# jeffersonfparil/poolgen

Hardware: AMD Instinct MI355X
Metric: loci/sec ols_iter_with_kinship, 200 pools x 10M loci (higher is better)
Workload: dtype f64

## Files before the change

### poolgen_amd/csrc/pg_kinship.hip

```cpp
#include "pg_common.h"
#include <cstdlib>
#include <cstring>
#include <utility>

namespace {

#ifndef KIN_WAVES_DEF
#define KIN_WAVES_DEF 16
#endif
constexpr int KIN_WAVES = KIN_WAVES_DEF;
constexpr int KIN_THREADS = 64 * KIN_WAVES;
#ifndef KIN_RING_D
#define KIN_RING_D 3
#endif
constexpr int KIN_FUSE_MAXK = 2;
constexpr int KIN_TPW = 96 / KIN_WAVES;
#ifndef KIN_KC_DEF
#define KIN_KC_DEF 16
#endif
constexpr int KIN_KC = KIN_KC_DEF;
constexpr int KIN_PPT = (KIN_KC * 128 + KIN_THREADS - 1) / KIN_THREADS;

typedef double double4_t __attribute__((ext_vector_type(4)));
typedef unsigned int uint4_t __attribute__((ext_vector_type(4)));

template <int CTRL, int ROW_MASK>
__device__ __forceinline__ double dpp_add(double v) {
    const int lo = __builtin_amdgcn_update_dpp(0, __double2loint(v), CTRL, ROW_MASK, 0xf, true);
    const int hi = __builtin_amdgcn_update_dpp(0, __double2hiint(v), CTRL, ROW_MASK, 0xf, true);
    return v + __hiloint2double(hi, lo);
}
template <int N>
__device__ __forceinline__ double row_from_plus(double v) {
    static_assert(N >= 1 && N <= 15, "row rotation");
    constexpr int CTRL = 0x120 + (16 - N);
    const int lo = __builtin_amdgcn_update_dpp(0, __double2loint(v), CTRL, 0xf, 0xf, false);
    const int hi = __builtin_amdgcn_update_dpp(0, __double2hiint(v), CTRL, 0xf, 0xf, false);
    return __hiloint2double(hi, lo);
}
template <int... I, typename F>
__device__ __forceinline__ void static_for_impl(std::integer_sequence<int, I...>, F &&f) {
    (f(std::integral_constant<int, I>{}), ...);
}
template <int N, typename F>
__device__ __forceinline__ void static_for(F &&f) {
    static_for_impl(std::make_integer_sequence<int, N>{}, f);
}
constexpr int kin_tri_ti(int t, int T) { int ti = 0; while (ti < T && t >= T - ti) { t -= T - ti; ++ti; } return ti < T ? ti : 0; }
constexpr int kin_tri_tj(int t, int T) { int ti = 0; while (ti < T && t >= T - ti) { t -= T - ti; ++ti; } return ti < T ? ti + t : 0; }
constexpr int kin_slot_tile(int w, int u, int T) { return (w + KIN_WAVES_DEF * u) < T * (T + 1) / 2 ? (w + KIN_WAVES_DEF * u) : 0; }

constexpr int KIN13_T[16][6][2] = {
    {{0, 0}, {0, 1}, {0, 2}, {1, 1}, {1, 2}, {2, 2}},
    {{3, 3}, {3, 4}, {3, 5}, {4, 4}, {4, 5}, {5, 5}},
    {{6, 6}, {6, 7}, {6, 8}, {7, 7}, {7, 8}, {8, 8}},
    {{9, 9}, {9, 10}, {9, 11}, {10, 10}, {10, 11}, {11, 11}},
    {{0, 3}, {0, 4}, {0, 5}, {1, 3}, {1, 4}, {1, 5}},
    {{0, 6}, {0, 7}, {0, 8}, {1, 6}, {1, 7}, {1, 8}},
    {{0, 9}, {0, 10}, {0, 11}, {1, 9}, {1, 10}, {1, 11}},
    {{3, 6}, {3, 7}, {3, 8}, {4, 6}, {4, 7}, {4, 8}},
    {{3, 9}, {3, 10}, {3, 11}, {4, 9}, {4, 10}, {4, 11}},
    {{6, 9}, {6, 10}, {6, 11}, {7, 9}, {7, 10}, {7, 11}},
    {{2, 4}, {2, 11}, {2, 12}, {4, 12}, {11, 12}, {12, 12}},
    {{2, 5}, {2, 6}, {2, 7}, {5, 6}, {5, 7}, {-1, -1}},
    {{0, 12}, {2, 3}, {3, 12}, {6, 12}, {7, 12}, {-1, -1}},
    {{5, 9}, {5, 10}, {5, 12}, {9, 12}, {10, 12}, {-1, -1}},
    {{2, 8}, {2, 9}, {2, 10}, {8, 9}, {8, 10}, {-1, -1}},
    {{1, 12}, {5, 8}, {5, 11}, {8, 11}, {8, 12}, {-1, -1}},
};
constexpr int kin13_ntiles(int w) { int c = 0; for (int u = 0; u < 6; ++u) c += KIN13_T[w][u][0] >= 0; return c; }
constexpr int kin13_col(int w, int idx) {
    int seen[12] = {-1, -1, -1, -1, -1, -1, -1, -1, -1, -1, -1, -1}, ns = 0;
    for (int u = 0; u < 6; ++u)
        for (int h = 0; h < 2; ++h) {
            const int c = KIN13_T[w][u][h];
            if (c < 0) continue;
            bool dup = false;
            for (int i = 0; i < ns; ++i) dup = dup || seen[i] == c;
            if (!dup) seen[ns++] = c;
        }
    return idx < ns ? seen[idx] : -1;
}
constexpr int kin13_ncols(int w) { int c = 0; while (c < 12 && kin13_col(w, c) >= 0) ++c; return c; }
constexpr int kin13_slot(int w, int col) { int i = 0; while (kin13_col(w, i) != col) ++i; return i; }
constexpr int KIN13_MAXC = 6;
constexpr int kin13_ndiag(int w) { int c = 0; for (int u = 0; u < 6; ++u) c += (KIN13_T[w][u][0] >= 0 && KIN13_T[w][u][0] == KIN13_T[w][u][1]); return c; }
constexpr int kin13_diag_index(int w, int u) { int c = 0; for (int v = 0; v < u; ++v) c += (KIN13_T[w][v][0] >= 0 && KIN13_T[w][v][0] == KIN13_T[w][v][1]); return c; }

struct KinParams {
    const double *G;
    int64_t p;
    int64_t ld;
    int64_t loci_per_wg;
    double *slabs;
    int n, T, npad, Tb, nb;
    int split;
    int merged;
    const double *ytil;
    double *spec;
    int k;
    int xcd_spx, npairs, nslab;
    int skip_dead;
    int wq_n[6], wq_first[6];
    int64_t wq_len[6];
};

template <bool FUSE, bool SPEC13, int SMALL = 0, bool SKIP = false>
__global__ __launch_bounds__(KIN_THREADS, 1) void k_kinship_syrk(KinParams P) {
    extern __shared__ __attribute__((aligned(16))) double lds[];
    const int tid = threadIdx.x;
    const int lane = tid & 63;
    const int wave = tid >> 6;
    const int fi = lane & 15;
    const int kq = lane >> 4;

    int bx = blockIdx.x, by = blockIdx.y;
    if (P.xcd_spx) {
        const int xcd = blockIdx.x & 7, s = blockIdx.x >> 3, main = P.xcd_spx * P.npairs;
        if (s < main) { bx = xcd * P.xcd_spx + s / P.npairs; by = s % P.npairs; }
        else { const int e = (s - main) * 8 + xcd; bx = 8 * P.xcd_spx + e / P.npairs; by = e % P.npairs; }
        if (bx >= P.nslab) return;
    }
    int64_t loci_per_wg = P.loci_per_wg;
    if (P.wq_n[0] > 0) {
        int q = 0;
        while (q + 1 < P.npairs && (int)blockIdx.x >= P.wq_first[q + 1]) ++q;
        by = q;
        bx = (int)blockIdx.x - P.wq_first[q];
        loci_per_wg = P.wq_len[q];
    }
    int bi = 0, bj = 0;
    {
        int q = by / P.split;
        const int first = P.merged ? 1 : 0;
        for (bi = 0; bi < P.nb; ++bi) {
            const int cnt = P.nb - bi - first;
            if (q < cnt) { bj = bi + first + q; break; }
            q -= cnt;
        }
    }
    const bool diag = (bi == bj);
    const int Ta = min(P.Tb, P.T - bi * P.Tb);
    const int Tbb = min(P.Tb, P.T - bj * P.Tb);
    const int colsA = Ta * 16;
    const int colsB = diag ? 0 : Tbb * 16;
    int ldsld = colsA + colsB;
    if ((ldsld & 31) != 16) ldsld += 16;
    const int a0 = bi * P.Tb * 16;
    const int b0 = bj * P.Tb * 16;
    const int wa = min(colsA, P.n - a0);
    const int wb = diag ? 0 : min(colsB, P.n - b0);
    const int npa = (wa + 1) >> 1, npb = (wb + 1) >> 1;
    const int npr = npa + npb;

    const int nrect = diag ? 0 : Ta * Tbb;
    const int NA = Ta * (Ta + 1) / 2, NB = Tbb * (Tbb + 1) / 2, part = P.nb - 1;
    const int rankA = bj - 1, rankB = bi;
    const int cntA = P.merged ? (NA > rankA ? (NA - rankA + part - 1) / part : 0) : 0;
    const int cntB = P.merged ? (NB > rankB ? (NB - rankB + part - 1) / part : 0) : 0;
    const int ntiles = diag ? NA : nrect + cntA + cntB;
    const int split_id = by % P.split;
    int acol[KIN_TPW], bcol[KIN_TPW], orow[KIN_TPW], ocol[KIN_TPW];
    bool live[KIN_TPW];
#pragma unroll
    for (int u = 0; u < KIN_TPW; ++u) {
        const int t = split_id + P.split * (wave + KIN_WAVES * u);
        int ti = 0, tj = 0;
        live[u] = t < ntiles;
        int kind = diag ? 1 : 0;
        if (t < ntiles) {
            int q = t, Td = Ta;
            if (!diag && t >= nrect) {
                const bool inA = t - nrect < cntA;
                kind = inA ? 1 : 2;
                q = inA ? rankA + part * (t - nrect) : rankB + part * (t - nrect - cntA);
                Td = inA ? Ta : Tbb;
            }
            if (kind) {
                for (ti = 0; ti < Td; ++ti) {
                    const int cnt = Td - ti;
                    if (q < cnt) { tj = ti + q; break; }
                    q -= cnt;
                }
            } else {
                ti = t / Tbb;
                tj = t - ti * Tbb;
            }
        }
        acol[u] = (kind == 2 ? colsA : 0) + 16 * ti;
        bcol[u] = (kind == 1 ? 0 : colsA) + 16 * tj;
        orow[u] = (kind == 2 ? b0 : a0) + 16 * ti;
        ocol[u] = (kind == 1 ? a0 : b0) + 16 * tj;
    }

    int st_loc[KIN_PPT], st_lcol[KIN_PPT];
    int st_gcol[KIN_PPT];
    bool st_on[KIN_PPT], st_two[KIN_PPT];
#pragma unroll
    for (int r = 0; r < KIN_PPT; ++r) {
        const int t = tid + r * KIN_THREADS;
        const int loc = t / npr;
        const int q = t - loc * npr;
        st_on[r] = loc < KIN_KC;
        st_loc[r] = loc;
        int gcol, lcol;
        bool two;
        if (q < npa) {
            gcol = a0 + 2 * q; lcol = 2 * q; two = (2 * q + 1) < wa;
        } else {
            const int q2 = q - npa;
            gcol = b0 + 2 * q2; lcol = colsA + 2 * q2; two = (2 * q2 + 1) < wb;
        }
        st_lcol[r] = lcol;
        st_two[r] = two;
        st_gcol[r] = st_on[r] ? gcol : a0;
        if (!st_on[r]) st_loc[r] = 0;
    }

    const int64_t l_begin = (int64_t)bx * loci_per_wg;
    const int64_t l_end = min(P.p, l_begin + loci_per_wg);
    const int nstages = (l_end > l_begin) ? (int)((l_end - l_begin + KIN_KC - 1) / KIN_KC) : 0;
    const int bufsz = KIN_KC * ldsld;

    for (int i = tid; i < 2 * bufsz; i += KIN_THREADS) lds[i] = 0.0;
    double *ylds = lds + 2 * bufsz;
    if (FUSE)
        for (int i = tid; i < P.k * 256; i += KIN_THREADS) ylds[i] = P.ytil[i];
    __syncthreads();

    const uint64_t slab_bytes64 = (uint64_t)(l_end > l_begin ? l_end - l_begin : 0) * P.ld * 8;
    const __amdgpu_buffer_rsrc_t rsrc = __builtin_amdgcn_make_buffer_rsrc(
        const_cast<double *>(P.G + l_begin * P.ld), 0, (int)(uint32_t)slab_bytes64, 0x00020000);
    uint4_t stage_reg[KIN_PPT];
    uint32_t st_voff[KIN_PPT];
#pragma unroll
    for (int r = 0; r < KIN_PPT; ++r)
        st_voff[r] = st_on[r] ? (uint32_t)(((int64_t)st_loc[r] * P.ld + st_gcol[r]) * 8) : 0xFFFFFFF0u;
    const uint32_t stage_stride = (uint32_t)(KIN_KC * P.ld * 8);
    auto stage_load = [&](int c) {
#pragma unroll
        for (int r = 0; r < KIN_PPT; ++r)
            stage_reg[r] = __builtin_amdgcn_raw_buffer_load_b128(
                rsrc, st_on[r] ? st_voff[r] + (uint32_t)c * stage_stride : 0xFFFFFFF0u, 0, 0);
    };
    auto stage_store = [&](int buf) {
#pragma unroll
        for (int r = 0; r < KIN_PPT; ++r) {
            if (st_on[r]) {
                uint4_t v = stage_reg[r];
                if (!st_two[r]) { v.z = 0u; v.w = 0u; }
                *reinterpret_cast<uint4_t *>(&lds[buf * bufsz + st_loc[r] * ldsld + st_lcol[r]]) = v;
            }
        }
    };

    if (nstages > 0) {
        stage_load(0);
        stage_store(0);
    }
    __syncthreads();

    const int NV = 2 + P.k;
    double *scratch = ylds + KIN_FUSE_MAXK * 256 + wave * (4 * 64);
    double yreg[KIN_FUSE_MAXK][4];
#pragma unroll
    for (int t = 0; t < KIN_FUSE_MAXK; ++t)
#pragma unroll
        for (int j = 0; j < 4; ++j) yreg[t][j] = (FUSE && t < P.k) ? ylds[t * 256 + lane + 64 * j] : 0.0;
    auto spec_pass = [&](const double *buf, int64_t lbase) {
#pragma unroll
        for (int jl = 0; jl < KIN_KC / KIN_WAVES; ++jl) {
            const int loc = wave + KIN_WAVES * jl;
            const double *row = buf + loc * ldsld;
            const double shift = row[0];
            double s1 = 0.0, s2 = 0.0, sy[KIN_FUSE_MAXK], d[4];
#pragma unroll
            for (int t = 0; t < KIN_FUSE_MAXK; ++t) sy[t] = 0.0;
#pragma unroll
            for (int j = 0; j < 4; ++j) {
                const int pool = lane + 64 * j;
                if (SPEC13 && j < 3) d[j] = row[pool] - shift;
                else {
                    const double gv = row[pool < ldsld ? pool : ldsld - 1];
                    d[j] = (pool < P.n) ? gv - shift : 0.0;
                }
                s1 += d[j];
                s2 = fma(d[j], d[j], s2);
                sy[0] = fma(d[j], yreg[0][j], sy[0]);
            }
            const bool two = P.k > 1;
            if (two) {
#pragma unroll
                for (int j = 0; j < 4; ++j) sy[1] = fma(d[j], yreg[1][j], sy[1]);
            }
            scratch[lane] = s1;
            scratch[64 + lane] = s2;
            scratch[2 * 64 + lane] = sy[0];
            if (two) scratch[3 * 64 + lane] = sy[1];
            __builtin_amdgcn_wave_barrier();
            const int v = lane >> 4, r = lane & 15;
            const double *sc = scratch + v * 64 + r;
            double tot = (sc[0] + sc[16]) + (sc[32] + sc[48]);
            tot = dpp_add<0x111, 0xf>(tot);
            tot = dpp_add<0x112, 0xf>(tot);
            tot = dpp_add<0x114, 0xf>(tot);
            tot = dpp_add<0x118, 0xf>(tot);
            const int64_t l = lbase + loc;
            if (r == 15 && v < NV && l < l_end) P.spec[l * NV + v] = tot;
            __builtin_amdgcn_wave_barrier();
        }
    };

    auto run = [&](auto wc, auto tc) {
        constexpr int W = decltype(wc)::value;
        constexpr int TPW = decltype(tc)::value;
        constexpr int KS = KIN_KC / 4;
        constexpr int NQ = KS * TPW;
        constexpr int D = KIN_RING_D, R = KIN_RING_D + 1;
        static_assert(NQ % R == 0 && NQ > 2 * D, "ring indexing assumes the stage length is a multiple of the ring");
        double4_t acc[TPW];
#pragma unroll
        for (int u = 0; u < TPW; ++u) acc[u] = (double4_t){0.0, 0.0, 0.0, 0.0};
#ifndef KIN_SHARED_FRAGS
#define KIN_SHARED_FRAGS 1
#endif
        if constexpr (W >= 0 && KIN_SHARED_FRAGS) {
            constexpr int NC = kin13_ncols(W), NT = kin13_ntiles(W);
            static_assert(NC <= KIN13_MAXC && KS % 2 == 0, "fragment sets alternate with the k-step parity");
            double fr[2][KIN13_MAXC];
            const double *lb = lds + kq * ldsld + fi;
            constexpr bool has_strip = [] { bool h = false; for (int u = 0; u < 6; ++u) h = h || (KIN13_T[W][u][0] >= 0 && KIN13_T[W][u][0] < 12 && KIN13_T[W][u][1] == 12); return h; }();
            double bs[2][2];
            const double *lbs = lds + kq * ldsld + 192 + (lane & 3);
            constexpr int ND = (SMALL & 1) ? kin13_ndiag(W) : 0;
            double bd[2][ND > 0 ? ND : 1][2];
            const double *lbr1 = lds + kq * ldsld + ((fi + 4) & 15), *lbr2 = lds + kq * ldsld + ((fi + 8) & 15);
            auto load_set = [&](const double *bufbase, auto sc, auto pc) __attribute__((always_inline)) {
                constexpr int s2 = decltype(sc)::value, par = decltype(pc)::value;
                static_for<NC>([&](auto cc) __attribute__((always_inline)) {
                    constexpr int ci = decltype(cc)::value;
                    fr[par][ci] = bufbase[4 * s2 * 208 + 16 * kin13_col(W, ci)];
                });
                if constexpr ((SMALL & 2) != 0 && has_strip) {
                    const double *bb = lbs + (bufbase - lb);
                    bs[par][0] = bb[4 * s2 * 208];
                    bs[par][1] = bb[4 * s2 * 208 + 4];
                }
                if constexpr (ND > 0) {
                    static_for<NT>([&](auto uc) __attribute__((always_inline)) {
                        constexpr int u = decltype(uc)::value;
                        if constexpr (KIN13_T[W][u][0] == KIN13_T[W][u][1]) {
                            constexpr int di = kin13_diag_index(W, u);
                            bd[par][di][0] = (lbr1 + (bufbase - lb))[4 * s2 * 208 + 16 * KIN13_T[W][u][0]];
                            bd[par][di][1] = (lbr2 + (bufbase - lb))[4 * s2 * 208 + 16 * KIN13_T[W][u][0]];
                        }
                    });
                }
            };
            auto mfma_set = [&](auto pc) __attribute__((always_inline)) {
                constexpr int par = decltype(pc)::value;
                static_for<NT>([&](auto uc) __attribute__((always_inline)) {
                    constexpr int u = decltype(uc)::value;
                    constexpr int ti = KIN13_T[W][u][0], tj = KIN13_T[W][u][1];
                    const double fa = fr[par][kin13_slot(W, ti)];
                    if constexpr ((SMALL & 1) != 0 && ti == tj) {
                        acc[u][0] = __builtin_amdgcn_mfma_f64_4x4x4f64(fa, fa, acc[u][0], 0, 0, 0);
                        acc[u][1] = __builtin_amdgcn_mfma_f64_4x4x4f64(fa, bd[par][kin13_diag_index(W, u)][0], acc[u][1], 0, 0, 0);
                        acc[u][2] = __builtin_amdgcn_mfma_f64_4x4x4f64(fa, bd[par][kin13_diag_index(W, u)][1], acc[u][2], 0, 0, 0);
                    } else if constexpr ((SMALL & 2) != 0 && tj == 12 && ti != tj) {
                        acc[u][0] = __builtin_amdgcn_mfma_f64_4x4x4f64(fa, bs[par][0], acc[u][0], 0, 0, 0);
                        acc[u][1] = __builtin_amdgcn_mfma_f64_4x4x4f64(fa, bs[par][1], acc[u][1], 0, 0, 0);
                    } else {
                        acc[u] = __builtin_amdgcn_mfma_f64_16x16x4f64(fa, fr[par][kin13_slot(W, tj)], acc[u], 0, 0, 0);
                    }
                });
            };
            if (nstages > 0) load_set(lb, std::integral_constant<int, 0>{}, std::integral_constant<int, 0>{});
            constexpr int spec_step = (W / 4) % KS;
            for (int c = 0; c < nstages; ++c) {
                const bool more = (c + 1) < nstages;
                if (more) stage_load(c + 1);
                const double *buf = lds + (c & 1) * bufsz;
                const double *b0 = lb + (c & 1) * bufsz;
                const double *b1 = lb + ((c + 1) & 1) * bufsz;
                static_for<KS>([&](auto sc) __attribute__((always_inline)) {
                    constexpr int s2 = decltype(sc)::value;
                    if constexpr (FUSE && s2 == spec_step) spec_pass(buf, l_begin + (int64_t)c * KIN_KC);
                    if constexpr (s2 + 1 < KS) {
                        load_set(b0, std::integral_constant<int, s2 + 1>{}, std::integral_constant<int, (s2 + 1) & 1>{});
                    } else {
                        if (more) stage_store((c + 1) & 1);
                        __syncthreads();
                        if (more) load_set(b1, std::integral_constant<int, 0>{}, std::integral_constant<int, 0>{});
                    }
                    mfma_set(std::integral_constant<int, s2 & 1>{});
                });
            }
            double *slab = P.slabs + (size_t)bx * P.npad * P.npad;
            static_for<NT>([&](auto uc) __attribute__((always_inline)) {
                constexpr int u = decltype(uc)::value;
                constexpr int ti = KIN13_T[W][u][0], tj = KIN13_T[W][u][1];
                constexpr int r0 = 16 * ti, c0 = 16 * tj;
                const int bi = lane >> 4, bb = (lane >> 2) & 3, bj = lane & 3;
                if constexpr ((SMALL & 1) != 0 && ti == tj) {
                    slab[(size_t)(r0 + 4 * bb + bi) * P.npad + c0 + 4 * bb + bj] = acc[u][0];
                    if (bb < 3) slab[(size_t)(r0 + 4 * bb + bi) * P.npad + c0 + 4 * (bb + 1) + bj] = acc[u][1];
                    else slab[(size_t)(r0 + bj) * P.npad + c0 + 12 + bi] = acc[u][1];
                    if (bb < 2) slab[(size_t)(r0 + 4 * bb + bi) * P.npad + c0 + 4 * (bb + 2) + bj] = acc[u][2];
                } else if constexpr ((SMALL & 2) != 0 && tj == 12 && ti != tj) {
                    slab[(size_t)(r0 + 4 * bb + bi) * P.npad + c0 + bj] = acc[u][0];
                    slab[(size_t)(r0 + 4 * bb + bi) * P.npad + c0 + 4 + bj] = acc[u][1];
                } else {
#pragma unroll
                    for (int r = 0; r < 4; ++r) slab[(size_t)(r0 + kq + 4 * r) * P.npad + c0 + fi] = acc[u][r];
                }
            });
            return;
        }
        double fa[R], fb[R];
        const double *lanebase = lds + kq * ldsld + fi;
        auto frag_load = [&](const double *bufbase, auto qc) {
            constexpr int q = decltype(qc)::value;
            constexpr int s = q / TPW, u = q % TPW;
            if constexpr (W >= 0) {
                if constexpr (W + KIN_WAVES * u >= 91) return;
                constexpr int t = kin_slot_tile(W, u, 13);
                constexpr int ao = 4 * s * 208 + 16 * kin_tri_ti(t, 13);
                constexpr int bo = 4 * s * 208 + 16 * kin_tri_tj(t, 13);
                fa[q % R] = bufbase[ao];
#ifdef KIN_EXP_HALF
                fb[q % R] = fa[q % R];
                (void)bo;
#elif defined(KIN_EXP_QUARTER)
                if constexpr (q % 2 == 0) fa[q % R] = bufbase[ao]; else fa[q % R] = fa[(q + R - 1) % R];
                fb[q % R] = fa[q % R];
                (void)bo;
#else
                fb[q % R] = bufbase[bo];
#endif
            } else {
                if constexpr (SKIP) { if (!live[u]) return; }
                const double *row = bufbase + 4 * s * ldsld;
                fa[q % R] = row[acol[u]];
                fb[q % R] = row[bcol[u]];
            }
        };
        auto mfma_item = [&](auto qc) {
            constexpr int q = decltype(qc)::value;
            constexpr int u = q % TPW;
            if constexpr (W >= 0 && W + KIN_WAVES * u >= 91) return;
            if constexpr (W < 0 && SKIP) { if (!live[u]) return; }
            acc[u] = __builtin_amdgcn_mfma_f64_16x16x4f64(fa[q % R], fb[q % R], acc[u], 0, 0, 0);
        };
        if (nstages > 0)
            static_for<D>([&](auto qc) { frag_load(lanebase, qc); });
        for (int c = 0; c < nstages; ++c) {
            const bool more = (c + 1) < nstages;
            if (more) stage_load(c + 1);
            const double *buf = lds + (c & 1) * bufsz;
            const double *fb0 = lanebase + (c & 1) * bufsz;
            const double *fb1 = lanebase + ((c + 1) & 1) * bufsz;
#ifndef KIN_SPEC_STAGGER
#define KIN_SPEC_STAGGER 1
#endif
            constexpr int spec_at = (FUSE && W >= 0 && KIN_SPEC_STAGGER) ? ((W / 4) % 4) * ((NQ - D) / 4) : -1;
            static_for<NQ - D>([&](auto qc) {
                if constexpr (decltype(qc)::value == spec_at) spec_pass(buf, l_begin + (int64_t)c * KIN_KC);
                frag_load(fb0, std::integral_constant<int, decltype(qc)::value + D>{});
                mfma_item(qc);
            });
            if (more) stage_store((c + 1) & 1);
            if (FUSE && spec_at < 0) spec_pass(buf, l_begin + (int64_t)c * KIN_KC);
            __syncthreads();
            static_for<D>([&](auto dc) {
                constexpr int q = NQ - D + decltype(dc)::value;
                if (more) frag_load(fb1, std::integral_constant<int, q + D - NQ>{});
                mfma_item(std::integral_constant<int, q>{});
            });
        }
        double *slab = P.slabs + (size_t)bx * P.npad * P.npad;
        static_for<TPW>([&](auto uc) {
            constexpr int u = decltype(uc)::value;
            bool on;
            int r0, c0;
            if constexpr (W >= 0) {
                constexpr int t = W + KIN_WAVES * u;
                on = t < 91;
                r0 = 16 * kin_tri_ti(kin_slot_tile(W, u, 13), 13);
                c0 = 16 * kin_tri_tj(kin_slot_tile(W, u, 13), 13);
            } else {
                on = live[u]; r0 = orow[u]; c0 = ocol[u];
            }
            if (on) {
#pragma unroll
                for (int r = 0; r < 4; ++r) slab[(size_t)(r0 + kq + 4 * r) * P.npad + c0 + fi] = acc[u][r];
            }
        });
    };
    if constexpr (SPEC13) {
        switch (wave) {
        case 0: run(std::integral_constant<int, 0>{}, std::integral_constant<int, KIN_TPW>{}); break;
        case 1: run(std::integral_constant<int, 1>{}, std::integral_constant<int, KIN_TPW>{}); break;
        case 2: run(std::integral_constant<int, 2>{}, std::integral_constant<int, KIN_TPW>{}); break;
        case 3: run(std::integral_constant<int, 3>{}, std::integral_constant<int, KIN_TPW>{}); break;
        case 4: run(std::integral_constant<int, 4>{}, std::integral_constant<int, KIN_TPW>{}); break;
        case 5: run(std::integral_constant<int, 5>{}, std::integral_constant<int, KIN_TPW>{}); break;
        case 6: run(std::integral_constant<int, 6>{}, std::integral_constant<int, KIN_TPW>{}); break;
#if KIN_WAVES_DEF == 8
        default: run(std::integral_constant<int, 7>{}, std::integral_constant<int, KIN_TPW>{}); break;
#else
        case 7: run(std::integral_constant<int, 7>{}, std::integral_constant<int, KIN_TPW>{}); break;
        case 8: run(std::integral_constant<int, 8>{}, std::integral_constant<int, KIN_TPW>{}); break;
        case 9: run(std::integral_constant<int, 9>{}, std::integral_constant<int, KIN_TPW>{}); break;
        case 10: run(std::integral_constant<int, 10>{}, std::integral_constant<int, KIN_TPW>{}); break;
        case 11: run(std::integral_constant<int, 11>{}, std::integral_constant<int, KIN_TPW>{}); break;
        case 12: run(std::integral_constant<int, 12>{}, std::integral_constant<int, KIN_TPW>{}); break;
        case 13: run(std::integral_constant<int, 13>{}, std::integral_constant<int, KIN_TPW>{}); break;
        case 14: run(std::integral_constant<int, 14>{}, std::integral_constant<int, KIN_TPW>{}); break;
        default: run(std::integral_constant<int, 15>{}, std::integral_constant<int, KIN_TPW>{}); break;
#endif
        }
    } else {
        constexpr std::integral_constant<int, -1> any{};
        switch ((ntiles + KIN_WAVES - 1) / KIN_WAVES) {
        case 0: case 1: case 2: run(any, std::integral_constant<int, 2>{}); break;
        case 3: run(any, std::integral_constant<int, 3>{}); break;
        case 4: run(any, std::integral_constant<int, 4>{}); break;
        case 5: run(any, std::integral_constant<int, 5>{}); break;
        default: run(any, std::integral_constant<int, KIN_TPW>{}); break;
        }
    }
}

constexpr double KIN_PAIR_FLOOR = 2.7;
struct KinCounts { int blk, nb, n[6]; };
__global__ __launch_bounds__(256) void k_kinship_reduce(const double *__restrict__ slabs, int nslabs, int npad, int n,
                                                        double add_const, double *__restrict__ S, const KinCounts C) {
    __shared__ double part[4][64];
    const int jj = threadIdx.x & 63, grp = threadIdx.x >> 6;
    const int j = blockIdx.x * 64 + jj;
    const int i = blockIdx.y;
    const bool on = i < n && j < n && i <= j;
    double s = 0.0;
    if (on && C.blk) {
        const int bi = i / C.blk, bj = j / C.blk;
        nslabs = C.n[bi * C.nb - bi * (bi - 1) / 2 + (bj - bi)];
    }
    if (on) {
        const size_t off = (size_t)i * npad + j;
        const size_t stride = (size_t)npad * npad;
        for (int w = grp; w < nslabs; w += 4) s += slabs[w * stride + off];
    }
    part[grp][jj] = s;
    __syncthreads();
    if (on && grp == 0) {
        const double t = ((part[0][jj] + part[1][jj]) + (part[2][jj] + part[3][jj])) + add_const;
        S[(size_t)i * n + j] = t;
        S[(size_t)j * n + i] = t;
    }
}

}

#ifndef KIN_LAUNCH_NAME
#define KIN_LAUNCH_NAME pg_launch_kinship
#endif
int KIN_LAUNCH_NAME(pg_ctx *ctx, const double *G, int64_t p, int n, int64_t ld, double *S,
                      bool add_intercept, int kid, bool allow_fuse) {
#if KIN_WAVES_DEF == 16
    if (n <= 64) return pg_launch_kinship_w8(ctx, G, p, n, ld, S, add_intercept, kid, allow_fuse);
#endif

    PG_CHECK(ctx, G && S, "kinship: null pointer");
    PG_CHECK(ctx, p > 0 && n > 0, "kinship: need p > 0 and n > 0 (p=%lld n=%d)", (long long)p, n);
    PG_CHECK(ctx, ld >= n && (ld % 2) == 0, "kinship: ld (%lld) must be even and >= n (%d)",
             (long long)ld, n);
    PG_CHECK(ctx, (reinterpret_cast<uintptr_t>(G) & 15) == 0, "kinship: G must be 16-byte aligned");
    PG_HIP(ctx, hipSetDevice(ctx->device));
    const int cus = ctx->cus;

    KinParams P;
    P.G = G; P.p = p; P.ld = ld; P.n = n;
    P.T = (n + 15) / 16;
    P.npad = P.T * 16;
    if (P.T <= 13) { P.Tb = P.T; P.nb = 1; }
    else { P.Tb = 8; P.nb = (P.T + 7) / 8; }
    P.merged = (P.nb >= 4 || (P.nb == 2 && P.T >= 15)) ? 1 : 0;
    if (!P.merged && P.nb >= 2 && P.nb <= 3) {
        double best = 1e30;
        int best_tb = P.Tb;
        for (int tb = (P.T + P.nb - 1) / P.nb; tb <= 8; ++tb) {
            double units = 0.0;
            for (int bi = 0; bi < P.nb; ++bi)
                for (int bj = bi; bj < P.nb; ++bj) {
                    const int Ta = std::min(tb, P.T - bi * tb), Tbb = std::min(tb, P.T - bj * tb);
                    if (Ta <= 0 || Tbb <= 0) { units += 1e6; continue; }
                    const int tiles = bi == bj ? Ta * (Ta + 1) / 2 : Ta * Tbb;
                    units += std::max(KIN_PAIR_FLOOR, (double)((tiles + KIN_WAVES - 1) / KIN_WAVES));
                }
            if (units <= best) { best = units; best_tb = tb; }
        }
        P.Tb = best_tb;
    }
    P.split = (P.merged && P.nb == 2) ? 2 : 1;
    const int npairs = (P.merged ? P.nb * (P.nb - 1) / 2 : P.nb * (P.nb + 1) / 2) * P.split;
    int nslab = cus / npairs;
    if (nslab < 1) nslab = 1;
    const int64_t max_slabs = (p + KIN_KC - 1) / KIN_KC;
    if (nslab > max_slabs) nslab = (int)max_slabs;
    P.loci_per_wg = (p + nslab - 1) / nslab;
    P.loci_per_wg = (P.loci_per_wg + KIN_KC - 1) / KIN_KC * KIN_KC;
    const int64_t max_loci_per_wg = ((int64_t)0xFFFFFFF0 / (ld * 8)) / KIN_KC * KIN_KC - KIN_KC;
    if (P.loci_per_wg > max_loci_per_wg) P.loci_per_wg = max_loci_per_wg;
    nslab = (int)((p + P.loci_per_wg - 1) / P.loci_per_wg);

    P.npairs = npairs; P.nslab = nslab;
    P.skip_dead = P.nb <= 2 ? 1 : 0;
    P.xcd_spx = 0;
    if (npairs > 1 && cus % 8 == 0) {
        const int spx = (cus / 8) / npairs;
        if (spx >= 1 && 8 * spx <= nslab) P.xcd_spx = spx;
    }
    for (int q = 0; q < 6; ++q) { P.wq_n[q] = 0; P.wq_first[q] = 0; P.wq_len[q] = 0; }
    KinCounts KC;
    KC.blk = 0; KC.nb = P.nb;
    for (int q = 0; q < 6; ++q) KC.n[q] = 0;
    int grid1d = 0;
    if (P.nb >= 2 && P.nb <= 3 && !P.merged) {
        double wgt[6], wsum = 0.0;
        int q = 0;
        for (int bi = 0; bi < P.nb; ++bi)
            for (int bj = bi; bj < P.nb; ++bj, ++q) {
                const int Ta = std::min(P.Tb, P.T - bi * P.Tb), Tbb = std::min(P.Tb, P.T - bj * P.Tb);
                const int tiles = bi == bj ? Ta * (Ta + 1) / 2 : Ta * Tbb;
                wgt[q] = std::max(KIN_PAIR_FLOOR, (double)((tiles + KIN_WAVES - 1) / KIN_WAVES)) + 0.35;
                wsum += wgt[q];
            }
        int used = 0;
        for (q = 0; q < npairs; ++q) { P.wq_n[q] = std::max(1, (int)(cus * wgt[q] / wsum)); used += P.wq_n[q]; }
        for (int left = cus - used; left > 0; --left) {
            int best = 0;
            for (q = 1; q < npairs; ++q)
                if (wgt[q] / P.wq_n[q] > wgt[best] / P.wq_n[best]) best = q;
            ++P.wq_n[best];
        }
        int first = 0, maxn = 0;
        for (q = 0; q < npairs; ++q) {
            int64_t len = (p + P.wq_n[q] - 1) / P.wq_n[q];
            len = (len + KIN_KC - 1) / KIN_KC * KIN_KC;
            if (len > max_loci_per_wg) len = max_loci_per_wg;
            P.wq_len[q] = len;
            P.wq_n[q] = (int)((p + len - 1) / len);
            P.wq_first[q] = first;
            first += P.wq_n[q];
            maxn = std::max(maxn, P.wq_n[q]);
            KC.n[q] = P.wq_n[q];
        }
        grid1d = first;
        nslab = maxn;
        P.nslab = nslab;
        P.xcd_spx = 0;
        P.skip_dead = 0;
        KC.blk = P.Tb * 16;
    }
    const size_t slab_bytes = (size_t)nslab * P.npad * P.npad * sizeof(double);
    int rc = pg_ws_reserve(ctx, slab_bytes);
    if (rc) return rc;
    P.slabs = static_cast<double *>(ctx->ws.get());

    int ldsld = (P.nb == 1) ? P.Tb * 16 : 2 * P.Tb * 16;
    if ((ldsld & 31) != 16) ldsld += 16;
    const size_t fuse_lds = (size_t)2 * KIN_KC * ldsld * 8 + ((size_t)KIN_FUSE_MAXK * 256 + (size_t)KIN_WAVES * 4 * 64) * 8;
    const bool fuse = allow_fuse && fuse_lds <= 160 * 1024 && P.nb == 1 && ctx->ph_n == n && ctx->ph_k >= 1 && ctx->ph_k <= KIN_FUSE_MAXK &&
                      ctx->ph_ytil_dev != nullptr;
    P.ytil = nullptr; P.spec = nullptr; P.k = 0;
    ctx->spec_valid = false;
    if (fuse) {
        const size_t need = (size_t)p * (2 + ctx->ph_k) * sizeof(double);
        const int rrc = ctx->spec_dev.reserve(ctx, need, "kinship");
        if (rrc) return rrc;
        P.ytil = ctx->ph_ytil_dev; P.spec = ctx->spec_dev; P.k = ctx->ph_k;
    }
    const size_t shmem = (size_t)2 * KIN_KC * ldsld * sizeof(double) + (fuse ? ((size_t)KIN_FUSE_MAXK * 256 + (size_t)KIN_WAVES * 4 * 64) * sizeof(double) : 0);
    const int max_cols = (P.nb == 1) ? P.Tb * 16 : 2 * P.Tb * 16;
    PG_CHECK(ctx, KIN_KC * (max_cols / 2) <= KIN_PPT * KIN_THREADS, "kinship: staging overflow");
    const bool spec13 = (P.nb == 1 && P.T == 13);
    auto launch = [&](auto kern) -> hipError_t {
        hipError_t e = hipFuncSetAttribute(reinterpret_cast<const void *>(kern),
                                           hipFuncAttributeMaxDynamicSharedMemorySize, (int)shmem);
        if (e != hipSuccess) return e;
        if (grid1d) hipLaunchKernelGGL(kern, dim3(grid1d), dim3(KIN_THREADS), shmem, ctx->stream, P);
        else if (P.xcd_spx) hipLaunchKernelGGL(kern, dim3(8 * ((P.xcd_spx * npairs) + ((nslab - 8 * P.xcd_spx) * npairs + 7) / 8)), dim3(KIN_THREADS), shmem,
                                          ctx->stream, P);
        else hipLaunchKernelGGL(kern, dim3(nslab, npairs), dim3(KIN_THREADS), shmem, ctx->stream, P);
        return hipSuccess;
    };
    pg_prof_begin(ctx, kid);
    hipError_t le;
    auto pick = [&](auto fz) -> hipError_t {
        constexpr bool FZ = decltype(fz)::value;
        if (!spec13) return P.skip_dead ? launch(k_kinship_syrk<FZ, false, 0, true>) : launch(k_kinship_syrk<FZ, false, 0, false>);
        return n <= 200 ? launch(k_kinship_syrk<FZ, true, 3>) : launch(k_kinship_syrk<FZ, true, 1>);
    };
    le = fuse ? pick(std::true_type{}) : pick(std::false_type{});
    PG_HIP(ctx, le);
    pg_prof_end(ctx);
    if (fuse) {
        ctx->spec_G = G; ctx->spec_p = p; ctx->spec_ld = ld; ctx->spec_n = n; ctx->spec_k = ctx->ph_k;
        ctx->spec_valid = true;
    }
    PG_HIP(ctx, hipGetLastError());
    pg_prof_begin(ctx, PG_K_KINSHIP_REDUCE);
    hipLaunchKernelGGL(k_kinship_reduce, dim3((n + 63) / 64, n), dim3(256), 0, ctx->stream,
                       P.slabs, nslab, P.npad, n, add_intercept ? 1.0 : 0.0, S, KC);
    pg_prof_end(ctx);
    PG_HIP(ctx, hipGetLastError());
    return PG_OK;
}

#ifndef KIN_NO_EXPORTS
extern "C" int pg_kinship_partial_dev(pg_ctx *ctx, const double *G_dev, int64_t p, int n,
                                      int64_t ld, double *S_dev) {
    if (!ctx) return PG_ERR_INVALID;
    return pg_launch_kinship(ctx, G_dev, p, n, ld, S_dev, false, PG_K_KINSHIP, true);
}

extern "C" int pg_gp_xxt_dev(pg_ctx *ctx, const double *G_dev, int64_t p, int n, int64_t ld,
                             double *XXt_dev) {
    if (!ctx) return PG_ERR_INVALID;
    return pg_launch_kinship(ctx, G_dev, p, n, ld, XXt_dev, true, PG_K_GP_XXT);
}

extern "C" int pg_set_phenotypes(pg_ctx *ctx, int n, const double *Y, int k) {
    if (!ctx) return PG_ERR_INVALID;
    ctx->spec_valid = false;
    if (n > 0 && Y && ctx->ph_n == n && ctx->ph_k == k && ctx->ph_ytil_dev && ctx->ph_Y.size() == (size_t)n * k &&
        std::memcmp(ctx->ph_Y.data(), Y, sizeof(double) * n * k) == 0)
        return PG_OK;
    ctx->ph_n = 0; ctx->ph_k = 0; ctx->ph_Y.clear();
    if (n == 0 || !Y) return PG_OK;
    PG_CHECK(ctx, n >= 2 && k >= 1, "set_phenotypes: bad shape n=%d k=%d", n, k);
    if (k > 4 || n > 256) return PG_OK;
    for (int i = 0; i < n * k; ++i)
        PG_CHECK(ctx, Y[i] == Y[i], "set_phenotypes: phenotype matrix contains NaN; remove pools with "
                                    "missing phenotypes first (gwas/ols.rs:287)");
    PG_HIP(ctx, hipSetDevice(ctx->device));
    std::vector<double> yt((size_t)k * 256, 0.0);
    for (int t = 0; t < k; ++t) {
        double mu = 0.0;
        for (int i = 0; i < n; ++i) mu += Y[(size_t)i * k + t];
        mu /= n;
        double syy = 0.0;
        for (int i = 0; i < n; ++i) {
            const double y = Y[(size_t)i * k + t] - mu;
            yt[(size_t)t * 256 + i] = y;
            syy += y * y;
        }
        ctx->ph_syy[t] = syy;
    }
    const int rc = ctx->ph_ytil_dev.reserve(ctx, sizeof(double) * 4 * 256, "set_phenotypes");
    if (rc) return rc;
    PG_HIP(ctx, hipMemcpyAsync(ctx->ph_ytil_dev, yt.data(), sizeof(double) * k * 256, hipMemcpyHostToDevice, ctx->stream));
    PG_HIP(ctx, hipStreamSynchronize(ctx->stream));
    ctx->ph_Y.assign(Y, Y + (size_t)n * k);
    ctx->ph_n = n; ctx->ph_k = k;
    return PG_OK;
}
#endif
```

Measured before the change: 1.259 billion.

## Compute fused per-locus statistics from MFMA fragments via owner waves and deferred reduction

In the fused kinship kernel with 13 tiles, the separate per-wave spec_pass over the LDS stage buffer is replaced. Owner waves that already hold full column fragments in registers now compute partial sums (sum, sum of squares, and y-products) as part of the MFMA k-step loop. They write these partials into a double-buffered LDS scratch area. A later stage reduces them across owners and with DPP lane adds. This removes redundant LDS reads and the serial spec pass from the inner loop, at the cost of more LDS, extra registers and a one-stage reduction lag.

```diff
diff --git a/poolgen_amd/csrc/pg_kinship.hip b/poolgen_amd/csrc/pg_kinship.hip
--- a/poolgen_amd/csrc/pg_kinship.hip
+++ b/poolgen_amd/csrc/pg_kinship.hip
@@ -12,6 +12,9 @@
 constexpr int KIN_THREADS = 64 * KIN_WAVES;
 #ifndef KIN_RING_D
 #define KIN_RING_D 3
+#endif
+#ifndef KIN_SHARED_FRAGS
+#define KIN_SHARED_FRAGS 1
 #endif
 constexpr int KIN_FUSE_MAXK = 2;
 constexpr int KIN_TPW = 96 / KIN_WAVES;
@@ -87,6 +90,33 @@
 constexpr int kin13_ndiag(int w) { int c = 0; for (int u = 0; u < 6; ++u) c += (KIN13_T[w][u][0] >= 0 && KIN13_T[w][u][0] == KIN13_T[w][u][1]); return c; }
 constexpr int kin13_diag_index(int w, int u) { int c = 0; for (int v = 0; v < u; ++v) c += (KIN13_T[w][v][0] >= 0 && KIN13_T[w][v][0] == KIN13_T[w][v][1]); return c; }
 
+
+constexpr int KIN13_OWNER[13] = {12, 15, 11, 12, 10, 13, 12, 11, 14, 13, 13, 15, 10};
+constexpr bool kin13_holds_full(int w, int col) {
+    for (int u = 0; u < 6; ++u) {
+        const int ti = KIN13_T[w][u][0], tj = KIN13_T[w][u][1];
+        if (ti < 0) continue;
+        if (ti == col || (tj == col && col != 12)) return true;
+    }
+    return false;
+}
+constexpr bool kin13_owners_ok() {
+    for (int c = 0; c < 13; ++c)
+        if (KIN13_OWNER[c] < 0 || KIN13_OWNER[c] >= 16 || !kin13_holds_full(KIN13_OWNER[c], c)) return false;
+    return true;
+}
+static_assert(kin13_owners_ok(), "every tile column needs one owner wave that holds its full fragment");
+constexpr int kin13_nown(int w) { int c = 0; for (int col = 0; col < 13; ++col) c += KIN13_OWNER[col] == w; return c; }
+constexpr int kin13_own_col(int w, int idx) { for (int col = 0; col < 13; ++col) if (KIN13_OWNER[col] == w && idx-- == 0) return col; return -1; }
+constexpr int kin13_owner_index(int w) { int c = 0; for (int v = 0; v < w; ++v) c += kin13_nown(v) > 0; return c; }
+constexpr int KIN13_NOWNERS = kin13_owner_index(16);
+constexpr int KIN13_NVAL = 2 + KIN_FUSE_MAXK;
+constexpr int KIN13_VP = (KIN_KC / 4) * 64 + 16;
+static_assert((KIN13_VP & 31) == 16, "scratch value pitch");
+constexpr int KIN13_OP = KIN13_NVAL * KIN13_VP;
+constexpr int KIN13_PP = KIN13_NOWNERS * KIN13_OP;
+constexpr int KIN13_STAGE = 2 * KIN_KC * 208;
+
 struct KinParams {
     const double *G;
     int64_t p;
@@ -223,8 +253,9 @@
     const int bufsz = KIN_KC * ldsld;
 
     for (int i = tid; i < 2 * bufsz; i += KIN_THREADS) lds[i] = 0.0;
+    constexpr bool OWNERS = FUSE && SPEC13 && KIN_SHARED_FRAGS;
     double *ylds = lds + 2 * bufsz;
-    if (FUSE)
+    if (FUSE && !OWNERS)
         for (int i = tid; i < P.k * 256; i += KIN_THREADS) ylds[i] = P.ytil[i];
     __syncthreads();
 
@@ -266,7 +297,7 @@
 #pragma unroll
     for (int t = 0; t < KIN_FUSE_MAXK; ++t)
 #pragma unroll
-        for (int j = 0; j < 4; ++j) yreg[t][j] = (FUSE && t < P.k) ? ylds[t * 256 + lane + 64 * j] : 0.0;
+        for (int j = 0; j < 4; ++j) yreg[t][j] = (FUSE && !OWNERS && t < P.k) ? ylds[t * 256 + lane + 64 * j] : 0.0;
     auto spec_pass = [&](const double *buf, int64_t lbase) {
 #pragma unroll
         for (int jl = 0; jl < KIN_KC / KIN_WAVES; ++jl) {
@@ -321,9 +352,6 @@
         double4_t acc[TPW];
 #pragma unroll
         for (int u = 0; u < TPW; ++u) acc[u] = (double4_t){0.0, 0.0, 0.0, 0.0};
-#ifndef KIN_SHARED_FRAGS
-#define KIN_SHARED_FRAGS 1
-#endif
         if constexpr (W >= 0 && KIN_SHARED_FRAGS) {
             constexpr int NC = kin13_ncols(W), NT = kin13_ntiles(W);
             static_assert(NC <= KIN13_MAXC && KS % 2 == 0, "fragment sets alternate with the k-step parity");
@@ -335,8 +363,20 @@
             constexpr int ND = (SMALL & 1) ? kin13_ndiag(W) : 0;
             double bd[2][ND > 0 ? ND : 1][2];
             const double *lbr1 = lds + kq * ldsld + ((fi + 4) & 15), *lbr2 = lds + kq * ldsld + ((fi + 8) & 15);
+            constexpr int NOWN = FUSE ? kin13_nown(W) : 0;
+            double yc[NOWN > 0 ? NOWN : 1][KIN_FUSE_MAXK];
+            double sh[2];
+            const bool in12 = FUSE && 192 + fi < P.n;
+            if constexpr (NOWN > 0) {
+                static_for<NOWN>([&](auto ic) __attribute__((always_inline)) {
+                    constexpr int i = decltype(ic)::value;
+#pragma unroll
+                    for (int t = 0; t < KIN_FUSE_MAXK; ++t) yc[i][t] = t < P.k ? P.ytil[t * 256 + 16 * kin13_own_col(W, i) + fi] : 0.0;
+                });
+            }
             auto load_set = [&](const double *bufbase, auto sc, auto pc) __attribute__((always_inline)) {
                 constexpr int s2 = decltype(sc)::value, par = decltype(pc)::value;
+                if constexpr (NOWN > 0) sh[par] = (bufbase - fi)[4 * s2 * 208];
                 static_for<NC>([&](auto cc) __attribute__((always_inline)) {
                     constexpr int ci = decltype(cc)::value;
                     fr[par][ci] = bufbase[4 * s2 * 208 + 16 * kin13_col(W, ci)];
@@ -375,26 +415,69 @@
                     }
                 });
             };
+            double *own_scr = NOWN > 0 ? lds + KIN13_STAGE + kin13_owner_index(W) * KIN13_OP + lane : nullptr;
+            auto own_step = [&](double *scr, auto sc) __attribute__((always_inline)) {
+                constexpr int s2 = decltype(sc)::value, par = s2 & 1;
+                double s1, sq, sy0, sy1;
+                static_for<NOWN>([&](auto ic) __attribute__((always_inline)) {
+                    constexpr int i = decltype(ic)::value;
+                    constexpr int col = kin13_own_col(W, i);
+                    double d = fr[par][kin13_slot(W, col)] - sh[par];
+                    if constexpr (col == 12) d = in12 ? d : 0.0;
+                    if constexpr (i == 0) { s1 = d; sq = d * d; sy0 = d * yc[i][0]; sy1 = d * yc[i][1]; }
+                    else { s1 += d; sq = fma(d, d, sq); sy0 = fma(d, yc[i][0], sy0); sy1 = fma(d, yc[i][1], sy1); }
+                });
+                scr[0 * KIN13_VP + 64 * s2] = s1;
+                scr[1 * KIN13_VP + 64 * s2] = sq;
+                scr[2 * KIN13_VP + 64 * s2] = sy0;
+                scr[3 * KIN13_VP + 64 * s2] = sy1;
+            };
+            const double *red_scr = FUSE ? lds + KIN13_STAGE + kq * KIN13_VP + fi : nullptr;
+            const bool red_lane = FUSE && fi == 15 && kq < NV;
+            auto reduce_stage = [&](const double *scr, int64_t lbase) __attribute__((always_inline)) {
+#pragma unroll
+                for (int jl = 0; jl < KIN_KC / KIN_WAVES; ++jl) {
+                    const int loc = W + KIN_WAVES * jl;
+                    const double *sc = scr + (loc / 4) * 64 + (loc % 4) * 16;
+                    double tot = sc[0];
+#pragma unroll
+                    for (int o = 1; o < KIN13_NOWNERS; ++o) tot += sc[o * KIN13_OP];
+                    tot = dpp_add<0x111, 0xf>(tot);
+                    tot = dpp_add<0x112, 0xf>(tot);
+                    tot = dpp_add<0x114, 0xf>(tot);
+                    tot = dpp_add<0x118, 0xf>(tot);
+                    const int64_t l = lbase + loc;
+                    if (l < l_end && red_lane) P.spec[l * NV + kq] = tot;
+                }
+            };
             if (nstages > 0) load_set(lb, std::integral_constant<int, 0>{}, std::integral_constant<int, 0>{});
-            constexpr int spec_step = (W / 4) % KS;
+            constexpr int spec_step = (W / 4 + 2) % KS;
+            int64_t red_l = l_end;
             for (int c = 0; c < nstages; ++c) {
                 const bool more = (c + 1) < nstages;
                 if (more) stage_load(c + 1);
-                const double *buf = lds + (c & 1) * bufsz;
                 const double *b0 = lb + (c & 1) * bufsz;
                 const double *b1 = lb + ((c + 1) & 1) * bufsz;
                 static_for<KS>([&](auto sc) __attribute__((always_inline)) {
                     constexpr int s2 = decltype(sc)::value;
-                    if constexpr (FUSE && s2 == spec_step) spec_pass(buf, l_begin + (int64_t)c * KIN_KC);
+                    if constexpr (FUSE && s2 == spec_step)
+                        reduce_stage(red_scr + ((c + 1) & 1) * KIN13_PP, red_l);
                     if constexpr (s2 + 1 < KS) {
                         load_set(b0, std::integral_constant<int, s2 + 1>{}, std::integral_constant<int, (s2 + 1) & 1>{});
+                        if constexpr (NOWN > 0) own_step(own_scr + (c & 1) * KIN13_PP, sc);
                     } else {
+                        if constexpr (NOWN > 0) own_step(own_scr + (c & 1) * KIN13_PP, sc);
                         if (more) stage_store((c + 1) & 1);
                         __syncthreads();
                         if (more) load_set(b1, std::integral_constant<int, 0>{}, std::integral_constant<int, 0>{});
                     }
                     mfma_set(std::integral_constant<int, s2 & 1>{});
                 });
+                red_l = l_begin + (int64_t)c * KIN_KC;
+            }
+            if constexpr (FUSE) {
+                __syncthreads();
+                reduce_stage(red_scr + ((nstages + 1) & 1) * KIN13_PP, red_l);
             }
             double *slab = P.slabs + (size_t)bx * P.npad * P.npad;
             static_for<NT>([&](auto uc) __attribute__((always_inline)) {
@@ -670,7 +753,9 @@
 
     int ldsld = (P.nb == 1) ? P.Tb * 16 : 2 * P.Tb * 16;
     if ((ldsld & 31) != 16) ldsld += 16;
-    const size_t fuse_lds = (size_t)2 * KIN_KC * ldsld * 8 + ((size_t)KIN_FUSE_MAXK * 256 + (size_t)KIN_WAVES * 4 * 64) * 8;
+    const bool spec13 = (P.nb == 1 && P.T == 13);
+    const size_t fuse_extra = (spec13 && KIN_SHARED_FRAGS ? (size_t)2 * KIN13_PP : (size_t)KIN_FUSE_MAXK * 256 + (size_t)KIN_WAVES * 4 * 64) * sizeof(double);
+    const size_t fuse_lds = (size_t)2 * KIN_KC * ldsld * sizeof(double) + fuse_extra;
     const bool fuse = allow_fuse && fuse_lds <= 160 * 1024 && P.nb == 1 && ctx->ph_n == n && ctx->ph_k >= 1 && ctx->ph_k <= KIN_FUSE_MAXK &&
                       ctx->ph_ytil_dev != nullptr;
     P.ytil = nullptr; P.spec = nullptr; P.k = 0;
@@ -681,10 +766,9 @@
         if (rrc) return rrc;
         P.ytil = ctx->ph_ytil_dev; P.spec = ctx->spec_dev; P.k = ctx->ph_k;
     }
-    const size_t shmem = (size_t)2 * KIN_KC * ldsld * sizeof(double) + (fuse ? ((size_t)KIN_FUSE_MAXK * 256 + (size_t)KIN_WAVES * 4 * 64) * sizeof(double) : 0);
+    const size_t shmem = fuse ? fuse_lds : (size_t)2 * KIN_KC * ldsld * sizeof(double);
     const int max_cols = (P.nb == 1) ? P.Tb * 16 : 2 * P.Tb * 16;
     PG_CHECK(ctx, KIN_KC * (max_cols / 2) <= KIN_PPT * KIN_THREADS, "kinship: staging overflow");
-    const bool spec13 = (P.nb == 1 && P.T == 13);
     auto launch = [&](auto kern) -> hipError_t {
         hipError_t e = hipFuncSetAttribute(reinterpret_cast<const void *>(kern),
                                            hipFuncAttributeMaxDynamicSharedMemorySize, (int)shmem);
```

Result: slower. 1.198 billion (-4.8%).
